# Sunscreen-tech/spf

Measured on NVIDIA B200. Metric: circuit_bootstraps_per_sec, higher is better.
Workload: dtype f64

## Files before the change

spf_b200/csrc/capi.cu:

```cuda
#include <cuda_runtime.h>
#include <math.h>
#include <stdio.h>
#include <stdlib.h>
#include <string.h>

#include <algorithm>
#include <atomic>
#include <chrono>
#include <condition_variable>
#include <map>
#include <memory>
#include <mutex>
#include <string>
#include <unordered_set>
#include <vector>

#include "../../include/spf_b200.h"
#include "kernels.cuh"
#include "tables.h"

using namespace spf;

namespace {

// ... 231 lines not shown
  }
  CUB(cudaStreamSynchronize(ctx->stream[0]));
#undef CUB
  *out = ctx;
  return 0;
}


int launch_pbs(spf_b200_ctx* ctx, uint64_t* d_glwe_out, const uint64_t* d_lwe_in, const uint64_t* d_lut, bool cbs,
               uint32_t log_chi, uint32_t log_v, size_t batch, cudaStream_t s, const void* const* ptrs = nullptr,
               bool packed = false) {
  if (batch == 0) return 0;
  PbsBatch P;
  P.lwe_in = d_lwe_in;
  P.lut = cbs ? nullptr : d_lut;
  P.lut_stride = 0;
  P.glwe_out = d_glwe_out;
  P.bsk = ctx->bsk;
  P.ptrs = ptrs;
  P.batch = (int)batch;
  P.lwe_n = (int)ctx->p.lwe_n;
  P.log_chi = (int)log_chi;
  P.log_v = (int)log_v;
  P.cbs_radix_log = (int)ctx->p.cbs.radix_log;
  P.cbs_count = (int)ctx->p.cbs.count;
  if (packed) {
    const int grid = (int)std::min<size_t>((batch + kPbsPairs - 1) / kPbsPairs, (size_t)ctx->sm_count);
    pbs_kernel<<<grid, kPbsPairs * 2 * kTeam, kPbsSmem, s>>>(P, tabs(ctx));
    return check_launch(ctx, "pbs_kernel");
  }
  if (batch <= (size_t)ctx->sm_count) {
    pbs_quad_kernel<<<(int)batch, 4 * kTeam, kQuadSmem, s>>>(P, tabs(ctx));
    return check_launch(ctx, "pbs_quad_kernel");
  }
  static const bool quad_tail = [] { const char* e = getenv("SPF_B200_PBS_TAIL"); return !(e && !strcmp(e, "pair")); }();
  const size_t wave = (size_t)ctx->sm_count * kPbsPairs;
  const size_t rem = batch % wave;
  if (quad_tail && batch > wave && rem > 0 && rem <= (size_t)ctx->sm_count && !P.lut_stride) {
    const size_t full = batch - rem;
    P.batch = (int)full;
    pbs_kernel<<<ctx->sm_count, kPbsPairs * 2 * kTeam, kPbsSmem, s>>>(P, tabs(ctx));
    if (int rc = check_launch(ctx, "pbs_kernel")) return rc;
    PbsBatch T = P;
    T.batch = (int)rem;
    T.glwe_out = d_glwe_out + full * 2 * kN;
    if (ptrs) T.ptrs = ptrs + full;
    else T.lwe_in = d_lwe_in + full * (size_t)(P.lwe_n + 1);
    pbs_quad_kernel<<<(int)rem, 4 * kTeam, kQuadSmem, s>>>(T, tabs(ctx));
    return check_launch(ctx, "pbs_quad_kernel");
  }
  const int per = per_cta(ctx, batch, kPbsPairs);
  const int grid = (int)std::min<size_t>((batch + per - 1) / per, (size_t)ctx->sm_count);
  pbs_kernel<<<grid, per * 2 * kTeam, kPbsSmem, s>>>(P, tabs(ctx));
  return check_launch(ctx, "pbs_kernel");
}

int launch_trace_ss(spf_b200_ctx* ctx, const uint64_t* d_glwe_in, uint64_t* d_glev_out, C2* d_ggsw_out, int mode,
                    int levels, double out_scale, size_t batch, cudaStream_t s, const void* const* ptrs = nullptr,
                    const PeerOffsets* peers = nullptr) {
  if (batch == 0) return 0;
  TraceSsBatch P;
  if (peers) P.peers = *peers;
  else P.peers.n = 0;
  P.glwe_in = d_glwe_in;
  P.glev_out = d_glev_out;
  P.ggsw_out = d_ggsw_out;
  P.ak = ctx->ak;
  P.ssk = ctx->ssk;
  P.kinv = ctx->kinv;
  P.ptrs = ptrs;
  P.batch = (int)batch;
  P.levels = levels;
  P.mode = mode;
  P.cbs_radix_log = (int)ctx->p.cbs.radix_log;
  P.cbs_count = (int)ctx->p.cbs.count;
  P.tr_radix_log = (int)ctx->p.tr.radix_log;
  P.tr_count = (int)ctx->p.tr.count;
  P.ss_radix_log = (int)ctx->p.ss.radix_log;
  P.ss_count = (int)ctx->p.ss.count;
  P.out_scale = out_scale;
  const size_t items = batch * (size_t)levels;
  const int per = per_cta(ctx, items, kTrTeams);
  const int grid = (int)((items + per - 1) / per);
  if (P.peers.n > 0) trace_ss_kernel<true><<<grid, per * kTeam, kTableBytes + per * kTrTeamBytes, s>>>(P, tabs(ctx));
  else trace_ss_kernel<false><<<grid, per * kTeam, kTableBytes + per * kTrTeamBytes, s>>>(P, tabs(ctx));
  return check_launch(ctx, "trace_ss_kernel");
}

int launch_cbs(spf_b200_ctx* ctx, C2* d_ggsw_out, uint64_t* d_glwe, const uint64_t* d_lwe_in, const void* const* ptrs,
               double out_scale, size_t batch, cudaStream_t s, const PeerOffsets* peers = nullptr) {
  if (batch == 0) return 0;
  static const bool overlap = [] { const char* e = getenv("SPF_B200_CBS_OVERLAP"); return !(e && !strcmp(e, "0")); }();
  const int levels = (int)ctx->p.cbs.count;
  const size_t wave = (size_t)ctx->sm_count * kPbsPairs, rem = batch % wave, full = batch - rem;
  const size_t lwe = (size_t)ctx->p.lwe_n + 1, ggsw = len_ggsw(&ctx->p, ctx->p.cbs);
  bool pays = false;
  if (full > 0 && rem > 0 && rem <= wave / 2) {
    const double c = 2.93e-4, sm = (double)ctx->sm_count;
    const double serial = (rem <= (size_t)ctx->sm_count ? 0.49 : 1.0) + (double)batch * c;
    const double tail_sms = (double)((rem + kPbsPairs - 1) / kPbsPairs);
    const double packed = std::max(1.0, ((double)full * c * sm + tail_sms) / sm) + (double)rem * c;
    pays = packed < serial;
  }
  if (!overlap || !pays || s == ctx->aux) {
    if (int rc = launch_pbs(ctx, d_glwe, d_lwe_in, nullptr, true, 0, cbs_log_v(&ctx->p), batch, s, ptrs)) return rc;
    return launch_trace_ss(ctx, d_glwe, nullptr, d_ggsw_out, 0, levels, out_scale, batch, s, nullptr, peers);
  }
  if (int rc = launch_pbs(ctx, d_glwe, d_lwe_in, nullptr, true, 0, cbs_log_v(&ctx->p), full, s, ptrs)) return rc;
  CU(cudaEventRecord(ctx->ev_cbs_main, s));
  CU(cudaStreamWaitEvent(ctx->aux, ctx->ev_cbs_main, 0));
  if (int rc = launch_pbs(ctx, d_glwe + full * 2 * kN, ptrs ? nullptr : d_lwe_in + full * lwe, nullptr, true, 0, cbs_log_v(&ctx->p), rem,
                          ctx->aux, ptrs ? ptrs + full : nullptr, true))
    return rc;
  CU(cudaEventRecord(ctx->ev_cbs_tail, ctx->aux));
  pause_kernel<<<1, 1, 0, s>>>(20000u);
  if (int rc = check_launch(ctx, "pause_kernel")) return rc;
  if (int rc = launch_trace_ss(ctx, d_glwe, nullptr, d_ggsw_out, 0, levels, out_scale, full, s, nullptr, peers)) return rc;
  CU(cudaStreamWaitEvent(s, ctx->ev_cbs_tail, 0));
  return launch_trace_ss(ctx, d_glwe + full * 2 * kN, nullptr, d_ggsw_out + full * ggsw, 0, levels, out_scale, rem, s, nullptr, peers);
}

int launch_cmux(spf_b200_ctx* ctx, uint64_t* d_out, const uint64_t* d_d0, const uint64_t* d_d1, const C2* d_ggsw,
                size_t ggsw_stride, int glwe_per_item, size_t n_glwe, cudaStream_t s, const void* const* ptrs = nullptr,
                void* const* out_ptrs = nullptr) {
  if (n_glwe == 0) return 0;
  CmuxBatch P;
  P.out_ptrs = out_ptrs;
  P.out = d_out;
  P.d0 = d_d0;
  P.d1 = d_d1;
  P.ggsw = d_ggsw;
  P.ggsw_stride = ggsw_stride;
  P.ptrs = ptrs;
  P.batch = (int)n_glwe;
  P.glwe_per_item = glwe_per_item;
  P.radix_log = (int)ctx->p.cbs.radix_log;
  P.count = (int)ctx->p.cbs.count;
  static const bool pdl = !getenv("SPF_B200_NO_PDL");
  cudaLaunchAttribute attr[1];
  attr[0].id = cudaLaunchAttributeProgrammaticStreamSerialization;
  attr[0].val.programmaticStreamSerializationAllowed = 1;
  cudaLaunchConfig_t cfg = {};
  cfg.stream = s;
  cfg.attrs = attr;
  cfg.numAttrs = pdl ? 1 : 0;
  const DevTables T = tabs(ctx);
  static const char* wide_env = getenv("SPF_B200_CMUX_WIDE_MAX");
  const size_t wide_max = wide_env ? (size_t)atoll(wide_env) : 2 * (size_t)ctx->sm_count;
  if (n_glwe <= wide_max && P.count == 4) {
    cfg.gridDim = dim3((unsigned)n_glwe);
    cfg.blockDim = dim3(kWideTeams * kTeam);
    cfg.dynamicSmemBytes = kWideSmem;
    cudaLaunchKernelEx(&cfg, cmux_wide_kernel, P, T);
    return check_launch(ctx, "cmux_wide_kernel");
  }
  const int per = per_cta(ctx, n_glwe, kCmuxTeams);
  cfg.gridDim = dim3((unsigned)((n_glwe + per - 1) / per));
  cfg.blockDim = dim3(per * kTeam);
  cfg.dynamicSmemBytes = kTableBytes + per * kCmuxTeamBytes;
  cudaLaunchKernelEx(&cfg, cmux_kernel, P, T);
  return check_launch(ctx, "cmux_kernel");
}

int launch_keyswitch(spf_b200_ctx* ctx, uint64_t* d_out, const uint64_t* d_in, size_t batch, cudaStream_t s,
                     const void* const* ptrs = nullptr, DevBuf* states = nullptr ) {
  if (batch == 0) return 0;
  KsBatch P;
  P.out = d_out;
// ... 538 lines not shown
```

spf_b200/csrc/emu.cpp:

```cpp
#include <pthread.h>
#include <stdlib.h>
#include <string.h>

#include <cmath>
#include <vector>

#include "tables.h"
#include "team_ops.cuh"

using namespace spf;

namespace {

struct HostCx {
  static constexpr bool kTmemTwiddles = false;
  int u;
  pthread_barrier_t* bar;
  void sync() { pthread_barrier_wait(bar); }
  uint64_t rp_stash[32];
  void rp_store(const uint64_t (&rp)[32]) { memcpy(rp_stash, rp, sizeof(rp_stash)); }
  void rp_load(uint64_t (&rp)[32]) { memcpy(rp, rp_stash, sizeof(rp_stash)); }
};

template <bool TR, bool CH>
struct HostPairCxT {
  static constexpr bool kTransient = TR;
  static constexpr bool kChunked = CH;
  int u, h;
  pthread_barrier_t* bar_half;
  pthread_barrier_t* bar_pair;
  static constexpr bool kTmemX1 = false;
  int time_index() const { return u; }
  void x1_fwd(C2 (&)[16]) {}
  void x1_inv(C2 (&)[16]) {}
  void sync() { pthread_barrier_wait(bar_half); }
  void pair_sync() { pthread_barrier_wait(bar_pair); }
  template <bool CONJ>
  void t1_mul(C2 (&v)[16], const C2* T1) {
    for (int k1 = 0; k1 < 16; k1++) v[k1] = CONJ ? cmul_conj(v[k1], T1[k1 * 64 + u]) : cmul(v[k1], T1[k1 * 64 + u]);
  }
  template <bool CONJ>
  void t2_mul(C2 (&v)[16], const C2* T2) {
    const int q = u >> 4;
    for (int k2 = 1; k2 < 16; k2++) v[k2] = CONJ ? cmul_conj(v[k2], T2[q * kT2Pad + k2]) : cmul(v[k2], T2[q * kT2Pad + k2]);
  }
  static constexpr bool kReaderT2 = true;
#ifndef SPF_PBS_TWOBUF
#define SPF_PBS_TWOBUF 0
#endif
  static constexpr bool kTwoBuf = SPF_PBS_TWOBUF != 0 && !CH;
#ifndef SPF_PBS_INT_CONV
#define SPF_PBS_INT_CONV 0
#endif
  static constexpr bool kIntConv = SPF_PBS_INT_CONV != 0;
#ifndef SPF_PBS_FRND_CONV
#define SPF_PBS_FRND_CONV 0
#endif
  static constexpr bool kFrndConv = SPF_PBS_FRND_CONV != 0;
  void rt2_fwd(double (&tw)[12], const C2* T2) { rt2_fwd_consts(T2, u >> 4, h, tw); }
  void rt2_inv(C2 (&w)[6], const C2* T2) { rt2_inv_consts(T2, u >> 4, h, w); }
  static constexpr bool kBskRing = false;
  const C2* bsk_acquire(int, const C2* g) { return g; }
  void bsk_release(int) {}
  void bsk_release_early(int) {}
  void bsk_skip(int) {}
  C2 bsk_load(const C2* p) { return *p; }
  static constexpr bool kFusedStores = CH;
  void sts(C2* p, C2 v) { *p = v; }
  template <bool CONJ>
  void t1_mul_store(C2 (&v)[16], const C2* T1, C2* buf) {
    for (int k1 = 0; k1 < 16; k1++) {
      v[k1] = CONJ ? cmul_conj(v[k1], T1[k1 * 64 + u]) : cmul(v[k1], T1[k1 * 64 + u]);
      buf[k1 * kXPad + u] = v[k1];
    }
  }
  template <bool CONJ>
  void t2_mul_store(C2 (&v)[16], const C2* T2, C2* buf) {
    const int k1 = u & 15, q = u >> 4;
    for (int k2 = 0; k2 < 16; k2++) {
      if (k2) v[k2] = CONJ ? cmul_conj(v[k2], T2[q * kT2Pad + k2]) : cmul(v[k2], T2[q * kT2Pad + k2]);
      buf[k1 * kXPad + q + 4 * k2] = v[k2];
    }
  }
  uint64_t own_stash[32];
  void own_load(uint64_t (&own)[32], const uint64_t*) { memcpy(own, own_stash, sizeof(own_stash)); }
  void own_store(const uint64_t (&own)[32]) { memcpy(own_stash, own, sizeof(own_stash)); }
  void own_ld8(uint64_t (&o)[8], int c) { memcpy(o, own_stash + 8 * c, 64); }
  void own_ld4x2(uint64_t (&o)[8], int m4) { memcpy(o, own_stash + m4, 32); memcpy(o + 4, own_stash + m4 + 16, 32); }
  void own_st4x2(const uint64_t (&o)[8], int m4) { memcpy(own_stash + m4, o, 32); memcpy(own_stash + m4 + 16, o + 4, 32); }
  void own_st_wait() {}
  void f_store(const C2 (&)[2][8]) {}
  void f_load(C2 (&)[2][8]) {}
};

template <class Cx, class Body>
struct PairLaunch {
  Body* body;
  Cx cx;
  static void* run(void* p) {
    PairLaunch* l = (PairLaunch*)p;
    (*l->body)(l->cx);
    return nullptr;
  }
};
// ... 270 lines not shown
```

spf_b200/csrc/kernels.cuh:

```cuda
#pragma once
#include <cuda_runtime.h>

#include "team_ops.cuh"

namespace spf {

__device__ __forceinline__ void tmem_ld16(uint32_t (&r)[16], uint32_t taddr);
__device__ __forceinline__ void tmem_st16(uint32_t taddr, const uint32_t (&r)[16]);
__device__ __forceinline__ void tmem_wait_ld();
__device__ __forceinline__ void tmem_wait_st();

struct DevCx {
  static constexpr bool kTmemTwiddles = false;
  int u;
  int bar;
  uint32_t rp_taddr;
  __device__ __forceinline__ void sync() const {
    asm volatile("bar.sync %0, 64;" ::"r"(bar) : "memory");
  }
  __device__ __forceinline__ void rp_store(const uint64_t (&rp)[32]) const {
#pragma unroll
    for (int c = 0; c < 4; c++) {
      uint32_t r[16];
#pragma unroll
// ... 867 lines not shown
        const C2 w1{__hiloint2double((int)r1[4 * i + 1], (int)r1[4 * i]), __hiloint2double((int)r1[4 * i + 3], (int)r1[4 * i + 2])};
        const int ka = 8 * half + i, kb = 8 * half + 4 + i;
        if (ka != 0) v[ka] = CONJ ? cmul_conj(v[ka], w0) : cmul(v[ka], w0);
        v[kb] = CONJ ? cmul_conj(v[kb], w1) : cmul(v[kb], w1);
      }
    }
#else
    const int q = u >> 4;
#pragma unroll
    for (int k2 = 1; k2 < 16; k2++) v[k2] = CONJ ? cmul_conj(v[k2], T2[q * kT2Pad + k2]) : cmul(v[k2], T2[q * kT2Pad + k2]);
#endif
  }
};

__global__ void __launch_bounds__(4 * kTeam, 1) pbs_quad_kernel(PbsBatch P, DevTables tabs) {
  extern __shared__ __align__(16) unsigned char smem[];
  C2* sT2 = reinterpret_cast<C2*>(smem);
  uint64_t* acc = reinterpret_cast<uint64_t*>(smem + kQuadT2Bytes);
  C2* xb = reinterpret_cast<C2*>(smem + kQuadT2Bytes + 2 * kN * 8);
  C2* row = reinterpret_cast<C2*>(smem + kQuadT2Bytes + 2 * kN * 8 + 4 * kXBuf * 16);
  uint64_t* mbar = reinterpret_cast<uint64_t*>(smem + kQuadT2Bytes + 2 * kN * 8 + 4 * kXBuf * 16 + kQuadRowBytes);
  C2* sT1 = row;
  load_tables(sT1, sT2, tabs);
  uint32_t tmem_alloc;
  const uint32_t t1_taddr = pair_tmem_init(sT1, sT2, tmem_alloc);
  if (threadIdx.x == 0) {
    asm volatile("mbarrier.init.shared::cta.b64 [%0], 1;" ::"r"(smem_u32(mbar)) : "memory");
    asm volatile("fence.mbarrier_init.release.cluster;" ::: "memory");
  }
  __syncthreads();
#if SPF_QUAD_READER_T2
  {
    const int tm = threadIdx.x / kTeam, uu = threadIdx.x % kTeam;
    double tw[6];
    C2 wi[3];
    rt2_group_consts(sT2, uu >> 4, 2 * (tm & 1) + (tm >> 1), tw, wi);
    const uint32_t base = t1_taddr + 448 + 24 * (tm >> 1);
#pragma unroll
    for (int i = 0; i < 3; i++)
      tmem_st4(base + 4 * i, (uint32_t)__double2loint(tw[2 * i]), (uint32_t)__double2hiint(tw[2 * i]), (uint32_t)__double2loint(tw[2 * i + 1]),
               (uint32_t)__double2hiint(tw[2 * i + 1]));
#pragma unroll
    for (int i = 0; i < 3; i++)
      tmem_st4(base + 12 + 4 * i, (uint32_t)__double2loint(wi[i].x), (uint32_t)__double2hiint(wi[i].x), (uint32_t)__double2loint(wi[i].y),
               (uint32_t)__double2hiint(wi[i].y));
    tmem_wait_st();
    asm volatile("tcgen05.fence::before_thread_sync;" ::: "memory");
    __syncthreads();
    asm volatile("tcgen05.fence::after_thread_sync;" ::: "memory");
  }
#endif
  const int team = threadIdx.x / kTeam;
  DevQuadCx cx{(int)(threadIdx.x % kTeam), team & 1, team >> 1, t1_taddr, row, mbar};
  int copies = 0;
  for (int c = blockIdx.x; c < P.batch; c += gridDim.x) {
    PbsArgs A;
    A.lwe_in = P.ptrs ? static_cast<const uint64_t*>(P.ptrs[c]) : P.lwe_in + (size_t)c * (P.lwe_n + 1);
    A.lut = P.lut ? P.lut + (size_t)c * P.lut_stride : nullptr;
    A.glwe_out = P.glwe_out + (size_t)c * 2 * kN;
    A.bsk = P.bsk;
    A.lwe_n = P.lwe_n;
    A.log_chi = P.log_chi;
    A.log_v = P.log_v;
    A.cbs_radix_log = P.cbs_radix_log;
    A.cbs_count = P.cbs_count;
    pbs_quad_team(cx, A, acc, xb, sT1, sT2, copies);
    cx.quad_sync();
  }
  pair_tmem_free(tmem_alloc);
}

#ifndef SPF_TR_TEAMS
#define SPF_TR_TEAMS 4
#endif
#ifndef SPF_TR_MIN_BLOCKS
#define SPF_TR_MIN_BLOCKS 1
#endif
#ifndef SPF_TR_TMEM_TW
#define SPF_TR_TMEM_TW 1
#endif
#ifndef SPF_TR_TW_PIPE
#define SPF_TR_TW_PIPE 0
#endif
struct DevTrCx : DevCx {
  static constexpr bool kTmemTwiddles = SPF_TR_TMEM_TW != 0;
  uint32_t tw_taddr;
#if SPF_TR_TW_PIPE
  template <bool CONJ, bool SKIP0>
  __device__ __forceinline__ void tw_mul(C2 (&v)[16], uint32_t base) const {
    uint32_t r[2][16];
    tmem_ld16(r[0], base);
    tmem_wait_ld();
#pragma unroll
    for (int g = 0; g < 4; g++) {
      if (g < 3) tmem_ld16(r[(g + 1) & 1], base + 16 * (g + 1));
#pragma unroll
      for (int i = 0; i < 4; i++) {
        const uint32_t* rr = r[g & 1];
        const C2 w{__hiloint2double((int)rr[4 * i + 1], (int)rr[4 * i]), __hiloint2double((int)rr[4 * i + 3], (int)rr[4 * i + 2])};
        const int k = 4 * g + i;
        if (!SKIP0 || k) v[k] = CONJ ? cmul_conj(v[k], w) : cmul(v[k], w);
      }
      if (g < 3) tmem_wait_ld();
    }
  }
  template <bool CONJ>
  __device__ __forceinline__ void t1_mul(C2 (&v)[16]) const { tw_mul<CONJ, false>(v, tw_taddr); }
  template <bool CONJ>
  __device__ __forceinline__ void t2_mul(C2 (&v)[16]) const { tw_mul<CONJ, true>(v, tw_taddr + 64); }
#else
  template <bool CONJ>
  __device__ __forceinline__ void t1_mul(C2 (&v)[16]) const {
#pragma unroll
    for (int g = 0; g < 4; g++) {
      uint32_t r[16];
      tmem_ld16(r, tw_taddr + 16 * g);
      tmem_wait_ld();
#pragma unroll
      for (int i = 0; i < 4; i++) {
        const C2 w{__hiloint2double((int)r[4 * i + 1], (int)r[4 * i]), __hiloint2double((int)r[4 * i + 3], (int)r[4 * i + 2])};
        const int k = 4 * g + i;
        v[k] = CONJ ? cmul_conj(v[k], w) : cmul(v[k], w);
      }
    }
  }
  template <bool CONJ>
  __device__ __forceinline__ void t2_mul(C2 (&v)[16]) const {
#pragma unroll
    for (int g = 0; g < 4; g++) {
      uint32_t r[16];
      tmem_ld16(r, tw_taddr + 64 + 16 * g);
      tmem_wait_ld();
#pragma unroll
      for (int i = 0; i < 4; i++) {
        const C2 w{__hiloint2double((int)r[4 * i + 1], (int)r[4 * i]), __hiloint2double((int)r[4 * i + 3], (int)r[4 * i + 2])};
        const int k = 4 * g + i;
        if (k) v[k] = CONJ ? cmul_conj(v[k], w) : cmul(v[k], w);
      }
    }
  }
#endif
};
constexpr int kTrTmemCols = SPF_TR_TMEM_TW ? 256 : 128;
constexpr int kTrTeams = SPF_TR_TEAMS;
constexpr int kTrTeamBytes = 2 * kN * 8 + kXBuf * 16;
constexpr int kTrSmem = kTableBytes + kTrTeams * kTrTeamBytes;

constexpr int kMaxPeers = 7;
struct PeerOffsets {
  int n;
  int rank_of[kMaxPeers];
  long long off[kMaxPeers];
};

struct TraceSsBatch {
  const uint64_t* glwe_in;
  uint64_t* glev_out;
  C2* ggsw_out;
  const C2* ak;
  const C2* ssk;
  const uint32_t* kinv;
  const void* const* ptrs;
  int batch, levels, mode;
  int cbs_radix_log, cbs_count, tr_radix_log, tr_count, ss_radix_log, ss_count;
  double out_scale;
  PeerOffsets peers;
};

template <bool PEERS>
__global__ void __launch_bounds__(kTrTeams * kTeam, SPF_TR_MIN_BLOCKS) trace_ss_kernel(const __grid_constant__ TraceSsBatch P, DevTables tabs) {
  extern __shared__ __align__(16) unsigned char smem[];
  C2* sT1 = reinterpret_cast<C2*>(smem);
  C2* sT2 = sT1 + kT1Elems;
  load_tables(sT1, sT2, tabs);
  __shared__ uint32_t tmem_base;
  const int warp = threadIdx.x >> 5;
  if (warp == 0) {
    asm volatile("tcgen05.alloc.cta_group::1.sync.aligned.shared::cta.b32 [%0], %1;" ::"r"(
                     (uint32_t)__cvta_generic_to_shared(&tmem_base)), "n"(kTrTmemCols) : "memory");
    asm volatile("tcgen05.relinquish_alloc_permit.cta_group::1.sync.aligned;" ::: "memory");
  }
  asm volatile("tcgen05.fence::before_thread_sync;" ::: "memory");
  __syncthreads();
  asm volatile("tcgen05.fence::after_thread_sync;" ::: "memory");
  const uint32_t tmem_alloc = tmem_base;
  const uint32_t tw_taddr = tmem_alloc + ((uint32_t)((warp & 3) * 32) << 16);
#if SPF_TR_TMEM_TW
  if (warp < 4) {
    const int uu = (warp & 1) * 32 + (threadIdx.x & 31);
#pragma unroll
    for (int k = 0; k < 16; k++) {
      const C2 w1 = sT1[k * 64 + uu];
      tmem_st4(tw_taddr + 4 * k, (uint32_t)__double2loint(w1.x), (uint32_t)__double2hiint(w1.x), (uint32_t)__double2loint(w1.y),
               (uint32_t)__double2hiint(w1.y));
      const C2 w2 = k ? sT2[(uu >> 4) * kT2Pad + k] : C2{1.0, 0.0};
      tmem_st4(tw_taddr + 64 + 4 * k, (uint32_t)__double2loint(w2.x), (uint32_t)__double2hiint(w2.x), (uint32_t)__double2loint(w2.y),
               (uint32_t)__double2hiint(w2.y));
    }
    tmem_wait_st();
  }
  asm volatile("tcgen05.fence::before_thread_sync;" ::: "memory");
  __syncthreads();
  asm volatile("tcgen05.fence::after_thread_sync;" ::: "memory");
#endif
  const int team = threadIdx.x / kTeam;
  const int item = blockIdx.x * (blockDim.x / kTeam) + team;
  if (item < P.batch * P.levels) {
    const int c = item / P.levels, level = item % P.levels;
    unsigned char* base = smem + kTableBytes + team * kTrTeamBytes;
    uint64_t* g = reinterpret_cast<uint64_t*>(base);
    C2* xbuf = reinterpret_cast<C2*>(base + 2 * kN * 8);
    DevTrCx cx;
    cx.u = (int)(threadIdx.x % kTeam);
    cx.bar = team + 1;
    cx.rp_taddr = tw_taddr + (SPF_TR_TMEM_TW ? 128u : 0u) + (uint32_t)(warp >> 2) * 64;
    cx.tw_taddr = tw_taddr;
    TraceSsArgs A;
    const size_t glwe = 2 * kN;
    if (P.ptrs) A.glwe_in = static_cast<const uint64_t*>(P.ptrs[c]) + (P.mode == 2 ? (size_t)level * glwe : 0);
    else if (P.mode == 0) A.glwe_in = P.glwe_in + (size_t)c * glwe;
    else A.glwe_in = P.glwe_in + (size_t)item * glwe;
    A.glev_out = P.glev_out ? P.glev_out + (size_t)item * glwe : nullptr;
    A.ggsw_out = P.ggsw_out ? P.ggsw_out + (size_t)c * 2 * P.cbs_count * 2 * kM : nullptr;
    A.ak = P.ak;
    A.ssk = P.ssk;
    A.kinv = P.kinv;
    A.level = level;
    A.mode = P.mode;
    A.cbs_radix_log = P.cbs_radix_log;
    A.cbs_count = P.cbs_count;
    A.tr_radix_log = P.tr_radix_log;
    A.tr_count = P.tr_count;
    A.ss_radix_log = P.ss_radix_log;
    A.ss_count = P.ss_count;
    A.out_scale = P.out_scale;
    A.n_peers = P.peers.n;
    A.peer_off = P.peers.off;
    trace_ss_team<PEERS>(cx, A, g, xbuf, sT1, sT2);
  }
  asm volatile("tcgen05.fence::before_thread_sync;" ::: "memory");
  __syncthreads();
  if (warp == 0) asm volatile("tcgen05.dealloc.cta_group::1.sync.aligned.b32 %0, %1;" ::"r"(tmem_alloc), "n"(kTrTmemCols) : "memory");
}

__global__ void peer_barrier_kernel(unsigned long long* flags, PeerOffsets peers, int rank, unsigned long long epoch, int* err,
                                    unsigned long long timeout_ns) {
  const int i = threadIdx.x;
  __threadfence_system();
  if (*reinterpret_cast<volatile int*>(err)) return;
  if (i < peers.n) {
    volatile unsigned long long* theirs = reinterpret_cast<unsigned long long*>(reinterpret_cast<char*>(flags) + peers.off[i]) + rank;
    *theirs = epoch;
    __threadfence_system();
    volatile unsigned long long* mine = flags + peers.rank_of[i];
    unsigned long long t0, t1;
    asm volatile("mov.u64 %0, %%globaltimer;" : "=l"(t0));
    while (*mine < epoch) {
      asm volatile("mov.u64 %0, %%globaltimer;" : "=l"(t1));
      if (t1 - t0 > timeout_ns) { atomicExch(err, 1); break; }
      __nanosleep(200);
    }
  }
  __threadfence_system();
}

__global__ void gather_outputs_kernel(unsigned long long* dst, const void* const* src, const unsigned long long* off8, const unsigned* n8) {
  const int k = blockIdx.y;
  const unsigned long long* s = static_cast<const unsigned long long*>(src[k]);
  unsigned long long* d = dst + off8[k];
  for (unsigned i = blockIdx.x * blockDim.x + threadIdx.x; i < n8[k]; i += gridDim.x * blockDim.x) d[i] = s[i];
}

__global__ void peer_bcast_kernel(const uint4* src, size_t n16, PeerOffsets peers) {
  for (size_t i = blockIdx.x * (size_t)blockDim.x + threadIdx.x; i < n16; i += (size_t)gridDim.x * blockDim.x) {
    const uint4 v = src[i];
    for (int r = 0; r < peers.n; r++)
      *reinterpret_cast<uint4*>(reinterpret_cast<char*>(const_cast<uint4*>(src + i)) + peers.off[r]) = v;
  }
}

constexpr int kBoxCopyMaxDst = 8;
struct BoxCopyItem {
  const unsigned long long* src;
  unsigned long long* dst[kBoxCopyMaxDst];
  unsigned n8;
  int n_dst;
};
template <int N>
struct BoxCopyTable {
  BoxCopyItem item[N];
};
constexpr int kBoxCopySmall = 32;
constexpr int kBoxCopyLarge = 400;
static_assert(sizeof(BoxCopyTable<kBoxCopyLarge>) <= 32764, "box copy table exceeds the kernel parameter limit");

template <int N>
__global__ void __launch_bounds__(256) box_copy_kernel(const __grid_constant__ BoxCopyTable<N> t) {
  const BoxCopyItem& it = t.item[blockIdx.y];
// ... 847 lines not shown
```

spf_b200/csrc/team_ops.cuh:

```cuda
#pragma once
#include <type_traits>

#include "fft16.cuh"

namespace spf {

constexpr double kInvM = 1.0 / 1024.0;

SPF_HD C2 ldg_c2(const C2* p) {
#if defined(__CUDA_ARCH__)
  const double2 t = __ldg(reinterpret_cast<const double2*>(p));
  return C2{t.x, t.y};
#else
  return *p;
#endif
}
SPF_HD C2 ldg_c2_pinned(const C2* p) {
#if defined(__CUDA_ARCH__)
  C2 r;
  asm volatile("ld.global.v2.f64 {%0, %1}, [%2];" : "=d"(r.x), "=d"(r.y) : "l"(p) : "memory");
  return r;
#else
  return *p;
#endif
// ... 34 lines not shown
SPF_HD void team_fft_inv(Cx& cx, C2 (&v)[16], C2* xbuf, const C2* T1, const C2* T2) {
  inv_pass3(v);
  cx.sync();
  inv_x2_write(v, xbuf, cx.u);
  cx.sync();
  inv_x2_read(v, xbuf, cx.u);
  if constexpr (Cx::kTmemTwiddles) {
    cx.template t2_mul<true>(v);
    dft16<true>(v);
  } else {
    inv_pass2(v, cx.u, T2);
  }
  inv_x1_write(v, xbuf, cx.u);
  cx.sync();
  inv_x1_read(v, xbuf, cx.u);
  if constexpr (Cx::kTmemTwiddles) {
    cx.template t1_mul<true>(v);
    inv_pass1_core(v);
  } else {
    inv_pass1(v, cx.u, T1);
  }
}

SPF_HD void mad_glwe(C2 (&acc)[2][16], const C2 (&v)[16], const C2* g, int u) {
#pragma unroll
  for (int h = 0; h < 4; h++) {
    C2 b0[4], b1[4];
#pragma unroll
    for (int i = 0; i < 4; i++) {
      b0[i] = ldg_c2(g + bin_of(u, 4 * h + i));
      b1[i] = ldg_c2(g + kM + bin_of(u, 4 * h + i));
    }
#pragma unroll
    for (int i = 0; i < 4; i++) {
      cmad(acc[0][4 * h + i], v[4 * h + i], b0[i]);
      cmad(acc[1][4 * h + i], v[4 * h + i], b1[i]);
    }
  }
}

SPF_HD void zero_acc(C2 (&acc)[2][16]) {
#pragma unroll
  for (int p = 0; p < 2; p++)
#pragma unroll
    for (int s = 0; s < 16; s++) acc[p][s] = C2{0.0, 0.0};
}

template <class Cx, class F>
SPF_HD void team_poly_fft(Cx& cx, C2 (&v)[16], F coef, C2* xbuf, const C2* T1, const C2* T2) {
#pragma unroll
  for (int m = 0; m < 16; m++) {
    v[m].x = i64_to_f64((int64_t)coef(cx.u + 64 * m));
    v[m].y = i64_to_f64((int64_t)coef(cx.u + 64 * m + kM));
  }
  team_fft_fwd(cx, v, xbuf, T1, T2);
#pragma unroll
  for (int s = 0; s < 16; s++) { v[s].x *= kInvM; v[s].y *= kInvM; }
}

template <class Cx, class F>
SPF_HD void state_init(Cx& cx, uint64_t* st, int radix_log, int count, F coef) {
#pragma unroll 4
  for (int i = 0; i < 32; i++) st[i * 64 + cx.u] = radix_round(coef(cx.u + 64 * i), radix_log, count);
}

template <class Cx>
SPF_HD void gadget_mad(Cx& cx, C2 (&acc)[2][16], uint64_t* st, C2* xbuf, const C2* T1, const C2* T2,
                       const C2* glev, int radix_log, int count) {
  for (int t = 0; t < count; t++) {
    C2 v[16];
#pragma unroll
    for (int m = 0; m < 16; m++) {
      uint64_t s0 = st[m * 64 + cx.u], s1 = st[(m + 16) * 64 + cx.u];
      v[m].x = i32_to_f64(next_digit(s0, radix_log));
      v[m].y = i32_to_f64(next_digit(s1, radix_log));
      st[m * 64 + cx.u] = s0;
      st[(m + 16) * 64 + cx.u] = s1;
    }
    team_fft_fwd(cx, v, xbuf, T1, T2);
    mad_glwe(acc, v, glev + (size_t)(count - 1 - t) * 2 * kM, cx.u);
  }
}

template <class Cx, class F>
SPF_HD void gadget_mad_stateless(Cx& cx, C2 (&acc)[2][16], F coef, C2* xbuf, const C2* T1, const C2* T2, const C2* glev,
                                 int radix_log, int count) {
  const uint64_t off = radix_offset(radix_log, count);
  const uint64_t dmask = (1ull << radix_log) - 1;
  const int32_t half = 1 << (radix_log - 1);
  {
    uint64_t rp[32];
#pragma unroll
    for (int i2 = 0; i2 < 32; i2++) rp[i2] = radix_round(coef(cx.u + 64 * i2), radix_log, count) + off;
    cx.rp_store(rp);
  }
  for (int t = 0; t < count; t++) {
    C2 v[16];
    {
      uint64_t rp[32];
      cx.rp_load(rp);
#pragma unroll
      for (int m = 0; m < 16; m++) {
        v[m].x = i32_to_f64((int32_t)((rp[m] >> (t * radix_log)) & dmask) - half);
        v[m].y = i32_to_f64((int32_t)((rp[m + 16] >> (t * radix_log)) & dmask) - half);
      }
    }
    team_fft_fwd(cx, v, xbuf, T1, T2);
    mad_glwe(acc, v, glev + (size_t)(count - 1 - t) * 2 * kM, cx.u);
  }
}

template <class Cx>
SPF_HD void cmux_team(Cx& cx, uint64_t* out, const uint64_t* d0, const uint64_t* d1, const C2* ggsw,
                      uint64_t* st, C2* xbuf, const C2* T1, const C2* T2, int radix_log, int count) {
  C2 acc[2][16];
  zero_acc(acc);
  for (int r = 0; r < 2; r++) {
    const uint64_t* a1 = d1 + r * kN;
    const uint64_t* a0 = d0 ? d0 + r * kN : nullptr;
    state_init(cx, st, radix_log, count,
               [&](int j) { return a0 ? ldg_u64(a1 + j) - ldg_u64(a0 + j) : ldg_u64(a1 + j); });
    gadget_mad(cx, acc, st, xbuf, T1, T2, ggsw + (size_t)r * count * 2 * kM, radix_log, count);
  }
#pragma unroll
  for (int p = 0; p < 2; p++) {
    team_fft_inv(cx, acc[p], xbuf, T1, T2);
#pragma unroll
    for (int m = 0; m < 16; m++) {
      const int j = cx.u + 64 * m;
      uint64_t re = f64_to_torus(acc[p][m].x), im = f64_to_torus(acc[p][m].y);
      if (d0) { re += ldg_u64(d0 + p * kN + j); im += ldg_u64(d0 + p * kN + j + kM); }
      out[p * kN + j] = re;
      out[p * kN + j + kM] = im;
    }
  }
}

struct PbsArgs {
  const uint64_t* lwe_in;
  const uint64_t* lut;
  uint64_t* glwe_out;
  const C2* bsk;
  int lwe_n;
  int log_chi, log_v;
  int cbs_radix_log, cbs_count;
};

SPF_HD uint32_t modulus_switch(uint64_t x, int log_chi, int log_v, int log_modulus) {
  const uint64_t mask = (1ull << log_modulus) - 1;
  x <<= log_chi;
  const int shift = 64 - (log_modulus - log_v);
  const uint64_t rnd = (x >> (shift - 1)) & 1;
  x >>= shift;
  return (uint32_t)(((x + rnd) & mask) << log_v);
}

SPF_HD uint64_t cbs_lut_coeff(int idx, int cbs_radix_log, int cbs_count, int v) {
  const int f = idx & (v - 1);
  if (f >= cbs_count) return 0;
  const int pb = cbs_radix_log * (f + 1) + 1;
  return pb < 64 ? 0 - (1ull << (64 - pb)) : 0;
}

template <bool INIT>
SPF_HD void mad_poly(C2 (&acc)[16], const C2 (&v)[16], const C2* g, int u) {
#pragma unroll
  for (int h = 0; h < 4; h++) {
    C2 b[4];
#pragma unroll
    for (int i = 0; i < 4; i++) b[i] = ldg_c2(g + bin_of(u, 4 * h + i));
#pragma unroll
    for (int i = 0; i < 4; i++) {
      if (INIT) acc[4 * h + i] = cmul(v[4 * h + i], b[i]);
      else cmad(acc[4 * h + i], v[4 * h + i], b[i]);
    }
  }
}
SPF_HD void mad_poly_shared(C2 (&acc)[16], const C2* dbuf, const C2* g, int u) {
#pragma unroll
  for (int h = 0; h < 4; h++) {
    C2 b[4], d[4];
#pragma unroll
    for (int i = 0; i < 4; i++) {
      b[i] = ldg_c2(g + bin_of(u, 4 * h + i));
      d[i] = dbuf[(4 * h + i) * 64 + u];
    }
#pragma unroll
    for (int i = 0; i < 4; i++) cmad(acc[4 * h + i], d[i], b[i]);
  }
}

// ... 642 lines not shown
#endif
  for (int i = 16 * t; i < 16 * t + 16; i++) {
    const int j = u + 64 * i;
    A.glwe_out[h * kN + j] = pa[j];
  }
}

SPF_HD void poly_to_torus(uint64_t (&r)[32], const C2 (&w)[16]) {
#pragma unroll
  for (int m4 = 0; m4 < 16; m4 += 4) {
    uint32_t mag_max = 0;
#pragma unroll
    for (int i = 0; i < 4; i++) {
      r[m4 + i] = f64_to_torus_impl<false, false>(w[m4 + i].x, 1.0, &mag_max);
      r[m4 + i + 16] = f64_to_torus_impl<false, false>(w[m4 + i].y, 1.0, &mag_max);
    }
    if (__builtin_expect(mag_max == kTorusCornerMag, 0)) {
#pragma unroll
      for (int i = 0; i < 4; i++) {
        r[m4 + i] = f64_to_torus(w[m4 + i].x);
        r[m4 + i + 16] = f64_to_torus(w[m4 + i].y);
      }
    }
  }
}

struct TraceSsArgs {
  const uint64_t* glwe_in;
  uint64_t* glev_out;
  C2* ggsw_out;
  const C2* ak;
  const C2* ssk;
  const uint32_t* kinv;
  int level;
  int mode;
  int cbs_radix_log, cbs_count;
  int tr_radix_log, tr_count;
  int ss_radix_log, ss_count;
  double out_scale;
  int n_peers;
  const long long* peer_off;
};

template <bool PEERS>
SPF_HD void ggsw_store(const TraceSsArgs& A, C2* p, C2 v) {
  *p = v;
  if (PEERS) {
#pragma unroll 1
    for (int r = 0; r < A.n_peers; r++) *reinterpret_cast<C2*>(reinterpret_cast<char*>(p) + A.peer_off[r]) = v;
  }
}

SPF_HD uint64_t automorph_coeff(const uint64_t* p, int j, uint32_t kinv) {
  const uint32_t i = ((uint32_t)j * kinv) & (2 * kN - 1);
  return i < (uint32_t)kN ? p[i] : 0 - p[i - kN];
}

template <bool PEERS = true, class Cx>
SPF_HD void trace_ss_team(Cx& cx, const TraceSsArgs& A, uint64_t* g , C2* xbuf, const C2* T1,
                          const C2* T2) {
  const int u = cx.u;
  if (A.mode == 0) {
    const int rot = (2 * kN - A.level) & (2 * kN - 1);
    for (int i = 0; i < 32; i++) {
      const int j = u + 64 * i;
      int idx = j - rot;
      bool neg = false;
      if (idx < 0) { idx += kN; neg = true; }
      if (idx < 0) { idx += kN; neg = false; }
      uint64_t ca = ldg_u64(A.glwe_in + idx), cb = ldg_u64(A.glwe_in + kN + idx);
      if (idx <= A.level) cb += 1ull << (64 - (A.cbs_radix_log * (idx + 1) + 1));
      if (neg) { ca = 0 - ca; cb = 0 - cb; }
      g[j] = (ca >> 11) + ((ca >> 10) & 1);
      g[kN + j] = (cb >> 11) + ((cb >> 10) & 1);
    }
  } else {
    for (int i = 0; i < 32; i++) {
      const int j = u + 64 * i;
      g[j] = ldg_u64(A.glwe_in + j);
      g[kN + j] = ldg_u64(A.glwe_in + kN + j);
    }
  }
  cx.sync();
  if (A.mode != 2) {
    for (int r = 0; r < 11; r++) {
      const uint32_t kinv = A.kinv[r];
      C2 f[2][16];
      zero_acc(f);
      gadget_mad_stateless(cx, f, [&](int j) { return automorph_coeff(g, j, kinv); }, xbuf, T1, T2,
                           A.ak + (size_t)r * A.tr_count * 2 * kM, A.tr_radix_log, A.tr_count);
      team_fft_inv(cx, f[1], xbuf, T1, T2);
      uint64_t db[32];
      poly_to_torus(db, f[1]);
#pragma unroll
      for (int m = 0; m < 16; m++) {
        const int j = u + 64 * m;
        db[m] = automorph_coeff(g + kN, j, kinv) - db[m];
        db[m + 16] = automorph_coeff(g + kN, j + kM, kinv) - db[m + 16];
      }
      team_fft_inv(cx, f[0], xbuf, T1, T2);
      cx.sync();
      {
        uint64_t da[32];
        poly_to_torus(da, f[0]);
#pragma unroll
        for (int m = 0; m < 16; m++) {
          const int j = u + 64 * m;
          g[j] -= da[m];
          g[j + kM] -= da[m + 16];
          g[kN + j] += db[m];
          g[kN + j + kM] += db[m + 16];
        }
      }
      cx.sync();
    }
    if (A.glev_out) {
      for (int i = 0; i < 32; i++) {
        const int j = u + 64 * i;
        A.glev_out[j] = g[j];
        A.glev_out[kN + j] = g[kN + j];
      }
    }
  }
  if (A.ggsw_out) {
    const size_t glwe_f = 2 * kM;
    C2* row0 = A.ggsw_out + ((size_t)0 * A.cbs_count + A.level) * glwe_f;
    C2* row1 = A.ggsw_out + ((size_t)1 * A.cbs_count + A.level) * glwe_f;
    C2 f[2][16];
    team_poly_fft(cx, f[0], [&](int j) { return g[kN + j]; }, xbuf, T1, T2);
#pragma unroll
    for (int s = 0; s < 16; s++) { ggsw_store<PEERS>(A, row1 + kM + bin_of(u, s), cscale(f[0][s], A.out_scale)); f[1][s] = C2{0.0, 0.0}; }
    gadget_mad_stateless(cx, f, [&](int j) { return g[j]; }, xbuf, T1, T2, A.ssk, A.ss_radix_log, A.ss_count);
#pragma unroll
    for (int s = 0; s < 16; s++) {
      ggsw_store<PEERS>(A, row0 + bin_of(u, s), cscale(f[0][s], A.out_scale));
      ggsw_store<PEERS>(A, row0 + kM + bin_of(u, s), cscale(f[1][s], A.out_scale));
    }
    team_poly_fft(cx, f[0], [&](int j) { return g[j]; }, xbuf, T1, T2);
#pragma unroll
    for (int s = 0; s < 16; s++) ggsw_store<PEERS>(A, row1 + bin_of(u, s), cscale(f[0][s], A.out_scale));
  }
}

constexpr int kWideTeams = 8;
#if defined(SPF_WIDE_TRACE) && defined(__CUDA_ARCH__)
#define SPF_WT(k) do { if (threadIdx.x == 0 && blockIdx.x == 0) wt[k] = clock64(); } while (0)
#else
#define SPF_WT(k) do { } while (0)
#endif
template <class Cx>
SPF_HD void cmux_wide(Cx& cx, uint64_t* out, const uint64_t* d0, const uint64_t* d1, const C2* ggsw, C2* xb,
                      const C2* T1, const C2* T2, int radix_log, int count) {
  const int u = cx.u, team = cx.team;
  const int r = team / count, t = team % count;
  C2* xown = xb + team * kXBuf;
#if defined(SPF_WIDE_TRACE) && defined(__CUDA_ARCH__)
  long long wt[8];
#endif
  SPF_WT(0);
  {
    const uint64_t off = radix_offset(radix_log, count);
    const uint64_t dmask = (1ull << radix_log) - 1;
    const int32_t half = 1 << (radix_log - 1);
    cx.template g_stage<0>();
    C2 v[16];
    const int shift = 64 - radix_log * count;
    if (shift >= 33) {
      const uint32_t c1 = (1u << (shift - 33)) + ((uint32_t)off << (shift - 32));
      const int sh = shift - 32 + t * radix_log;
#pragma unroll
      for (int m = 0; m < 16; m++) {
        if (m == 8) cx.template g_stage<1>();
        const int j = r * kN + u + 64 * m;
        const uint64_t x0 = d0 ? d1[j] - d0[j] : d1[j];
        const uint64_t x1 = d0 ? d1[j + kM] - d0[j + kM] : d1[j + kM];
        v[m].x = i32_to_f64((int32_t)((((uint32_t)(x0 >> 32) + c1) >> sh) & (uint32_t)dmask) - half);
        v[m].y = i32_to_f64((int32_t)((((uint32_t)(x1 >> 32) + c1) >> sh) & (uint32_t)dmask) - half);
      }
    } else {
      cx.template g_stage<1>();
#pragma unroll
      for (int m = 0; m < 16; m++) {
        const int j = r * kN + u + 64 * m;
        const uint64_t x0 = d0 ? d1[j] - d0[j] : d1[j];
        const uint64_t x1 = d0 ? d1[j + kM] - d0[j + kM] : d1[j + kM];
        const uint64_t r0 = radix_round(x0, radix_log, count) + off, r1 = radix_round(x1, radix_log, count) + off;
        v[m].x = i32_to_f64((int32_t)((r0 >> (t * radix_log)) & dmask) - half);
        v[m].y = i32_to_f64((int32_t)((r1 >> (t * radix_log)) & dmask) - half);
      }
    }
    SPF_WT(1);
    cx.template g_stage<2>();
    fwd_pass1_core(v);
    cx.template g_stage<3>();
#pragma unroll
    for (int k1i = 0; k1i < 16; k1i++) v[k1i] = cmul(v[k1i], T1[k1i * 64 + u]);
    cx.template g_stage<4>();
    fwd_x1_write(v, xown, u);
    cx.sync();
    SPF_WT(2);
    fwd_x1_read(v, xown, u);
    cx.template g_stage<5>();
    dft16<false>(v);
    cx.template g_stage<6>();
    {
      const int qq = u >> 4;
#pragma unroll
      for (int k2i = 1; k2i < 16; k2i++) v[k2i] = cmul(v[k2i], T2[qq * kT2Pad + k2i]);
    }
    cx.template g_stage<7>();
    fwd_x2_write(v, xown, u);
    cx.template g_stage<8>();
  }
  cx.cta_sync();
  SPF_WT(3);
// ... 66 lines not shown
```

Baseline: 57910.

## Add TMA key ring and TMEM accumulator parking to trace kernel; drop smem tables

When twiddles live in tensor memory (the default), the trace/scheme-switch kernel no longer stages twiddle tables in shared memory. It fills its tensor-memory twiddles straight from global memory and starts team buffers at offset zero, which cuts shared memory per CTA and removes the table-load prologue. Two opt-in paths are added behind compile flags. One streams automorphism and scheme-switch key chunks into a two-stage shared-memory ring with cp.async.bulk and mbarriers, released by a cross-warp counter. The other parks the GLWE accumulators in tensor memory to relieve register pressure. Both opt-in paths add synchronisation complexity and carry a risk of deadlock or hazards.

```diff
diff --git a/spf_b200/csrc/capi.cu b/spf_b200/csrc/capi.cu
--- a/spf_b200/csrc/capi.cu
+++ b/spf_b200/csrc/capi.cu
@@ -337,8 +337,8 @@
   const size_t items = batch * (size_t)levels;
   const int per = per_cta(ctx, items, kTrTeams);
   const int grid = (int)((items + per - 1) / per);
-  if (P.peers.n > 0) trace_ss_kernel<true><<<grid, per * kTeam, kTableBytes + per * kTrTeamBytes, s>>>(P, tabs(ctx));
-  else trace_ss_kernel<false><<<grid, per * kTeam, kTableBytes + per * kTrTeamBytes, s>>>(P, tabs(ctx));
+  if (P.peers.n > 0) trace_ss_kernel<true><<<grid, per * kTeam, kTrTeamsOff + per * kTrTeamBytes, s>>>(P, tabs(ctx));
+  else trace_ss_kernel<false><<<grid, per * kTeam, kTrTeamsOff + per * kTrTeamBytes, s>>>(P, tabs(ctx));
   return check_launch(ctx, "trace_ss_kernel");
 }
 
diff --git a/spf_b200/csrc/emu.cpp b/spf_b200/csrc/emu.cpp
--- a/spf_b200/csrc/emu.cpp
+++ b/spf_b200/csrc/emu.cpp
@@ -20,6 +20,12 @@
   uint64_t rp_stash[32];
   void rp_store(const uint64_t (&rp)[32]) { memcpy(rp_stash, rp, sizeof(rp_stash)); }
   void rp_load(uint64_t (&rp)[32]) { memcpy(rp, rp_stash, sizeof(rp_stash)); }
+  static constexpr bool kKeyChunks = true;
+  static constexpr bool kParkF = false;
+  void f_get(C2 (&)[16], int) {}
+  const C2* key_acquire(int, const C2* g) { return g; }
+  void key_release(int) {}
+  C2 key_load(const C2* p) { return *p; }
 };
 
 template <bool TR, bool CH>
diff --git a/spf_b200/csrc/kernels.cuh b/spf_b200/csrc/kernels.cuh
--- a/spf_b200/csrc/kernels.cuh
+++ b/spf_b200/csrc/kernels.cuh
@@ -973,9 +973,130 @@
 #ifndef SPF_TR_TW_PIPE
 #define SPF_TR_TW_PIPE 0
 #endif
+#ifndef SPF_TR_RING
+#define SPF_TR_RING 0
+#endif
+#ifndef SPF_TR_TMEM_F
+#define SPF_TR_TMEM_F 0
+#endif
+static_assert(!SPF_TR_RING || SPF_TR_TMEM_TW, "the trace key ring takes the place of the twiddle tables: the twiddles must live in tensor memory");
+constexpr int kTrRingStages = 2;
+constexpr int kTrChunkBytes = kM * 16;
 struct DevTrCx : DevCx {
   static constexpr bool kTmemTwiddles = SPF_TR_TMEM_TW != 0;
+  static constexpr bool kKeyChunks = SPF_TR_RING || SPF_TR_TMEM_F;
   uint32_t tw_taddr;
+  uint32_t ring_s = 0, full_s = 0;
+  unsigned* rel = nullptr;
+  const C2* ak = nullptr;
+  const C2* ssk = nullptr;
+  int tr_count = 0, ss_count = 0;
+  int n_tr = 0, total = 0, nwarps = 0;
+  __device__ __forceinline__ const C2* key_src(int G) const {
+    const int p = G & 1;
+    if (G < n_tr) {
+      const int k = G >> 1, r = k / tr_count, t = k % tr_count;
+      return ak + ((size_t)(r * tr_count + tr_count - 1 - t) * 2 + p) * kM;
+    }
+    const int t = (G - n_tr) >> 1;
+    return ssk + ((size_t)(ss_count - 1 - t) * 2 + p) * kM;
+  }
+  __device__ __forceinline__ void ring_issue(int G) const {
+    const uint32_t st = (uint32_t)(G % kTrRingStages);
+    asm volatile("fence.proxy.async.shared::cta;" ::: "memory");
+    asm volatile("mbarrier.arrive.expect_tx.shared::cta.b64 _, [%0], %1;" ::"r"(full_s + 8 * st), "r"((uint32_t)kTrChunkBytes) : "memory");
+    asm volatile("cp.async.bulk.shared::cluster.global.mbarrier::complete_tx::bytes [%0], [%1], %2, [%3];"
+                 ::"r"(ring_s + st * kTrChunkBytes), "l"(key_src(G)), "r"((uint32_t)kTrChunkBytes), "r"(full_s + 8 * st) : "memory");
+  }
+  __device__ __forceinline__ const C2* key_acquire(int G, const C2* g) const {
+#if SPF_TR_RING
+    const int st = G % kTrRingStages;
+    mbar_wait_trap(full_s + 8 * st, (uint32_t)(G / kTrRingStages) & 1u);
+    __syncwarp();
+    return reinterpret_cast<const C2*>((size_t)(ring_s + st * kTrChunkBytes));
+#else
+    return g;
+#endif
+  }
+  __device__ __forceinline__ C2 key_load(const C2* p) const {
+#if SPF_TR_RING
+    C2 r;
+    asm volatile("ld.shared.v2.f64 {%0, %1}, [%2];" : "=d"(r.x), "=d"(r.y) : "r"((uint32_t)(size_t)p) : "memory");
+    return r;
+#else
+    return ldg_c2(p);
+#endif
+  }
+  __device__ __forceinline__ void key_release(int G) const {
+#if SPF_TR_RING
+    __syncwarp();
+    if ((threadIdx.x & 31) == 0) {
+      const int st = G % kTrRingStages;
+      __threadfence_block();
+      if (atomicAdd(rel + st, 1u) == (unsigned)nwarps - 1u) {
+        atomicExch(rel + st, 0u);
+        __threadfence_block();
+        if (G + kTrRingStages < total) ring_issue(G + kTrRingStages);
+      }
+    }
+#endif
+  }
+  static constexpr bool kParkF = SPF_TR_TMEM_F != 0;
+  uint32_t f_taddr;
+  __device__ __forceinline__ void f_park(const C2 (&acc)[2][16]) const {
+#pragma unroll
+    for (int c = 0; c < 8; c++) {
+      uint32_t r[16];
+#pragma unroll
+      for (int i = 0; i < 4; i++) {
+        const C2 a = acc[c >> 2][4 * (c & 3) + i];
+        r[4 * i] = (uint32_t)__double2loint(a.x);
+        r[4 * i + 1] = (uint32_t)__double2hiint(a.x);
+        r[4 * i + 2] = (uint32_t)__double2loint(a.y);
+        r[4 * i + 3] = (uint32_t)__double2hiint(a.y);
+      }
+      tmem_st16(f_taddr + 16 * c, r);
+    }
+    tmem_wait_st();
+  }
+  __device__ __forceinline__ void f_get(C2 (&a)[16], int p) const {
+    if constexpr (kParkF) {
+#pragma unroll
+      for (int c = 0; c < 4; c++) {
+        uint32_t r[16];
+        tmem_ld16(r, f_taddr + 64 * p + 16 * c);
+        tmem_wait_ld();
+#pragma unroll
+        for (int i = 0; i < 4; i++)
+          a[4 * c + i] = C2{__hiloint2double((int)r[4 * i + 1], (int)r[4 * i]), __hiloint2double((int)r[4 * i + 3], (int)r[4 * i + 2])};
+      }
+    }
+  }
+  __device__ __forceinline__ void f_mad(int p, const C2 (&v)[16], const C2* h) const {
+#pragma unroll
+    for (int q = 0; q < 2; q++) {
+      uint32_t r[2][16];
+      tmem_ld16(r[0], f_taddr + 64 * p + 32 * q);
+      tmem_ld16(r[1], f_taddr + 64 * p + 32 * q + 16);
+      C2 b[8];
+#pragma unroll
+      for (int i = 0; i < 8; i++) b[i] = key_load(h + bin_of(u, 8 * q + i));
+      tmem_wait_ld();
+#pragma unroll
+      for (int i = 0; i < 8; i++) {
+        uint32_t* w = &r[i >> 2][4 * (i & 3)];
+        C2 a{__hiloint2double((int)w[1], (int)w[0]), __hiloint2double((int)w[3], (int)w[2])};
+        cmad(a, v[8 * q + i], b[i]);
+        w[0] = (uint32_t)__double2loint(a.x);
+        w[1] = (uint32_t)__double2hiint(a.x);
+        w[2] = (uint32_t)__double2loint(a.y);
+        w[3] = (uint32_t)__double2hiint(a.y);
+      }
+      tmem_st16(f_taddr + 64 * p + 32 * q, r[0]);
+      tmem_st16(f_taddr + 64 * p + 32 * q + 16, r[1]);
+    }
+    tmem_wait_st();
+  }
 #if SPF_TR_TW_PIPE
   template <bool CONJ, bool SKIP0>
   __device__ __forceinline__ void tw_mul(C2 (&v)[16], uint32_t base) const {
@@ -1032,10 +1153,15 @@
   }
 #endif
 };
-constexpr int kTrTmemCols = SPF_TR_TMEM_TW ? 256 : 128;
+constexpr int kTrTmemRp = SPF_TR_TMEM_TW ? 128 : 0;
+constexpr int kTrTmemF = kTrTmemRp + 128;
+constexpr int kTrTmemCols = SPF_TR_TMEM_F ? 512 : kTrTmemF;
 constexpr int kTrTeams = SPF_TR_TEAMS;
 constexpr int kTrTeamBytes = 2 * kN * 8 + kXBuf * 16;
-constexpr int kTrSmem = kTableBytes + kTrTeams * kTrTeamBytes;
+constexpr int kTrRingBytes = kTrRingStages * kTrChunkBytes;
+constexpr int kTrTeamsOff = SPF_TR_RING ? kTrRingBytes + 64 : SPF_TR_TMEM_TW ? 0 : kTableBytes;
+constexpr int kTrSmem = kTrTeamsOff + kTrTeams * kTrTeamBytes;
+static_assert(kTrSmem <= 232448, "trace_ss_kernel shared memory");
 
 constexpr int kMaxPeers = 7;
 struct PeerOffsets {
@@ -1061,9 +1187,14 @@
 template <bool PEERS>
 __global__ void __launch_bounds__(kTrTeams * kTeam, SPF_TR_MIN_BLOCKS) trace_ss_kernel(const __grid_constant__ TraceSsBatch P, DevTables tabs) {
   extern __shared__ __align__(16) unsigned char smem[];
+#if SPF_TR_TMEM_TW
+  const C2* sT1 = nullptr;
+  const C2* sT2 = nullptr;
+#else
   C2* sT1 = reinterpret_cast<C2*>(smem);
   C2* sT2 = sT1 + kT1Elems;
   load_tables(sT1, sT2, tabs);
+#endif
   __shared__ uint32_t tmem_base;
   const int warp = threadIdx.x >> 5;
   if (warp == 0) {
@@ -1081,10 +1212,10 @@
     const int uu = (warp & 1) * 32 + (threadIdx.x & 31);
 #pragma unroll
     for (int k = 0; k < 16; k++) {
-      const C2 w1 = sT1[k * 64 + uu];
+      const C2 w1 = tabs.T1[k * 64 + uu];
       tmem_st4(tw_taddr + 4 * k, (uint32_t)__double2loint(w1.x), (uint32_t)__double2hiint(w1.x), (uint32_t)__double2loint(w1.y),
                (uint32_t)__double2hiint(w1.y));
-      const C2 w2 = k ? sT2[(uu >> 4) * kT2Pad + k] : C2{1.0, 0.0};
+      const C2 w2 = k ? tabs.T2[(uu >> 4) * kT2Pad + k] : C2{1.0, 0.0};
       tmem_st4(tw_taddr + 64 + 4 * k, (uint32_t)__double2loint(w2.x), (uint32_t)__double2hiint(w2.x), (uint32_t)__double2loint(w2.y),
                (uint32_t)__double2hiint(w2.y));
     }
@@ -1095,16 +1226,43 @@
   asm volatile("tcgen05.fence::after_thread_sync;" ::: "memory");
 #endif
   const int team = threadIdx.x / kTeam;
-  const int item = blockIdx.x * (blockDim.x / kTeam) + team;
+  const int per = blockDim.x / kTeam;
+  const int item = blockIdx.x * per + team;
+  DevTrCx cx;
+#if SPF_TR_RING
+  {
+    uint64_t* full = reinterpret_cast<uint64_t*>(smem + kTrRingBytes);
+    cx.ring_s = smem_u32(smem);
+    cx.full_s = smem_u32(full);
+    cx.rel = reinterpret_cast<unsigned*>(full + kTrRingStages);
+    cx.ak = P.ak;
+    cx.ssk = P.ssk;
+    cx.tr_count = P.tr_count;
+    cx.ss_count = P.ss_count;
+    cx.n_tr = P.mode != 2 ? 2 * 11 * P.tr_count : 0;
+    cx.total = cx.n_tr + (P.ggsw_out ? 2 * P.ss_count : 0);
+    cx.nwarps = 2 * min(per, P.batch * P.levels - (int)blockIdx.x * per);
+    if (threadIdx.x == 0) {
+      for (int st = 0; st < kTrRingStages; st++) {
+        asm volatile("mbarrier.init.shared::cta.b64 [%0], 1;" ::"r"(cx.full_s + 8 * st) : "memory");
+        cx.rel[st] = 0;
+      }
+      asm volatile("fence.mbarrier_init.release.cluster;" ::: "memory");
+    }
+    __syncthreads();
+    if (threadIdx.x == 0)
+      for (int g0 = 0; g0 < kTrRingStages && g0 < cx.total; g0++) cx.ring_issue(g0);
+  }
+#endif
   if (item < P.batch * P.levels) {
     const int c = item / P.levels, level = item % P.levels;
-    unsigned char* base = smem + kTableBytes + team * kTrTeamBytes;
+    unsigned char* base = smem + kTrTeamsOff + team * kTrTeamBytes;
     uint64_t* g = reinterpret_cast<uint64_t*>(base);
     C2* xbuf = reinterpret_cast<C2*>(base + 2 * kN * 8);
-    DevTrCx cx;
     cx.u = (int)(threadIdx.x % kTeam);
     cx.bar = team + 1;
-    cx.rp_taddr = tw_taddr + (SPF_TR_TMEM_TW ? 128u : 0u) + (uint32_t)(warp >> 2) * 64;
+    cx.rp_taddr = tw_taddr + kTrTmemRp + (uint32_t)(warp >> 2) * 64;
+    cx.f_taddr = tw_taddr + kTrTmemF + (uint32_t)(warp >> 2) * 128;
     cx.tw_taddr = tw_taddr;
     TraceSsArgs A;
     const size_t glwe = 2 * kN;
diff --git a/spf_b200/csrc/team_ops.cuh b/spf_b200/csrc/team_ops.cuh
--- a/spf_b200/csrc/team_ops.cuh
+++ b/spf_b200/csrc/team_ops.cuh
@@ -140,9 +140,15 @@
   }
 }
 
+template <class Cx>
+SPF_HD void mad_half(Cx& cx, C2 (&acc)[16], const C2 (&v)[16], const C2* h) {
+#pragma unroll
+  for (int s = 0; s < 16; s++) cmad(acc[s], v[s], cx.key_load(h + bin_of(cx.u, s)));
+}
+
 template <class Cx, class F>
 SPF_HD void gadget_mad_stateless(Cx& cx, C2 (&acc)[2][16], F coef, C2* xbuf, const C2* T1, const C2* T2, const C2* glev,
-                                 int radix_log, int count) {
+                                 int radix_log, int count, int& K) {
   const uint64_t off = radix_offset(radix_log, count);
   const uint64_t dmask = (1ull << radix_log) - 1;
   const int32_t half = 1 << (radix_log - 1);
@@ -152,6 +158,7 @@
     for (int i2 = 0; i2 < 32; i2++) rp[i2] = radix_round(coef(cx.u + 64 * i2), radix_log, count) + off;
     cx.rp_store(rp);
   }
+  if constexpr (Cx::kParkF) cx.f_park(acc);
   for (int t = 0; t < count; t++) {
     C2 v[16];
     {
@@ -164,7 +171,18 @@
       }
     }
     team_fft_fwd(cx, v, xbuf, T1, T2);
-    mad_glwe(acc, v, glev + (size_t)(count - 1 - t) * 2 * kM, cx.u);
+    const C2* row = glev + (size_t)(count - 1 - t) * 2 * kM;
+    if constexpr (Cx::kKeyChunks) {
+#pragma unroll
+      for (int p = 0; p < 2; p++) {
+        const C2* h = cx.key_acquire(K, row + p * kM);
+        if constexpr (Cx::kParkF) cx.f_mad(p, v, h);
+        else mad_half(cx, acc[p], v, h);
+        cx.key_release(K++);
+      }
+    } else {
+      mad_glwe(acc, v, row, cx.u);
+    }
   }
 }
 
@@ -973,13 +991,15 @@
     }
   }
   cx.sync();
+  int K = 0;
   if (A.mode != 2) {
     for (int r = 0; r < 11; r++) {
       const uint32_t kinv = A.kinv[r];
       C2 f[2][16];
       zero_acc(f);
       gadget_mad_stateless(cx, f, [&](int j) { return automorph_coeff(g, j, kinv); }, xbuf, T1, T2,
-                           A.ak + (size_t)r * A.tr_count * 2 * kM, A.tr_radix_log, A.tr_count);
+                           A.ak + (size_t)r * A.tr_count * 2 * kM, A.tr_radix_log, A.tr_count, K);
+      cx.f_get(f[1], 1);
       team_fft_inv(cx, f[1], xbuf, T1, T2);
       uint64_t db[32];
       poly_to_torus(db, f[1]);
@@ -989,6 +1009,7 @@
         db[m] = automorph_coeff(g + kN, j, kinv) - db[m];
         db[m + 16] = automorph_coeff(g + kN, j + kM, kinv) - db[m + 16];
       }
+      cx.f_get(f[0], 0);
       team_fft_inv(cx, f[0], xbuf, T1, T2);
       cx.sync();
       {
@@ -1021,7 +1042,9 @@
     team_poly_fft(cx, f[0], [&](int j) { return g[kN + j]; }, xbuf, T1, T2);
 #pragma unroll
     for (int s = 0; s < 16; s++) { ggsw_store<PEERS>(A, row1 + kM + bin_of(u, s), cscale(f[0][s], A.out_scale)); f[1][s] = C2{0.0, 0.0}; }
-    gadget_mad_stateless(cx, f, [&](int j) { return g[j]; }, xbuf, T1, T2, A.ssk, A.ss_radix_log, A.ss_count);
+    gadget_mad_stateless(cx, f, [&](int j) { return g[j]; }, xbuf, T1, T2, A.ssk, A.ss_radix_log, A.ss_count, K);
+    cx.f_get(f[0], 0);
+    cx.f_get(f[1], 1);
 #pragma unroll
     for (int s = 0; s < 16; s++) {
       ggsw_store<PEERS>(A, row0 + bin_of(u, s), cscale(f[0][s], A.out_scale));
```

Result: no change. 57830, median of 6 (-0.1%).
